# pgvector/pgvector

Measured on AMD Instinct MI355X. Metric: QPS @ recall@10 (IVFFlat, 1M x 1536d), higher is better.
Workload: dtype f32

## Files before the change

include/pgv_hip.h:

```cpp
#ifndef PGV_HIP_H
#define PGV_HIP_H

#include <stddef.h>
#include <stdint.h>

#ifdef __cplusplus
extern "C" {
#endif

#define PGV_ABI_VERSION 1

#define PGV_OK 0
#define PGV_ERR_ARG 1
#define PGV_ERR_DIMS 2
#define PGV_ERR_DEVICE 3
#define PGV_ERR_NOMEM 4
#define PGV_ERR_STATE 5
#define PGV_ERR_DATA 6

typedef enum pgv_dtype
{
	PGV_F32 = 0,
	PGV_F16 = 1
}			pgv_dtype;
// ... 51 lines not shown
	double		scan_pairs;
	double		scan_rows;
	double		aux_ms;
	int64_t		aux_launches;
	double		aux_pairs;
	double		assign_redo_rows;
	double		assign_rows;
	double		assign_recheck_rows;
	double		scan_unique_rows;
	double		scan_redo_queries;
	double		scan_widened_queries;
	double		scan_shadow_queries;
}			pgv_stats;
int			pgv_ctx_set_profiling(pgv_ctx * ctx, int on);
int			pgv_ctx_set_exact_scan(pgv_ctx * ctx, int on);
#define PGV_BOUND_STATISTICAL 0
#define PGV_BOUND_WORST_CASE 1
int			pgv_ctx_set_bound(pgv_ctx * ctx, int mode);
int			pgv_ctx_reset_stats(pgv_ctx * ctx);
int			pgv_ctx_get_stats(pgv_ctx * ctx, pgv_stats * out);


int			pgv_index_upload(pgv_ctx * ctx, pgv_metric metric, pgv_dtype dtype, int dim, int nlists,
							 const void *centers, const int64_t *list_offsets,
							 const void *vectors, const uint64_t *tids, pgv_index * *out);
void		pgv_index_free(pgv_index * index);
int			pgv_index_share(pgv_index * index, pgv_ctx * ctx, pgv_index * *out);
int			pgv_index_set_overlap(pgv_index * index, int lanes);
#define PGV_INDEX_HANDLE_BYTES 256
typedef struct pgv_index_handle
// ... 5 lines not shown
int			pgv_index_tids(pgv_index * index, const int64_t *slots, int64_t n, uint64_t *out);
int64_t		pgv_index_rows(const pgv_index * index);
int			pgv_index_lists(const pgv_index * index);

int			pgv_rank_lists(pgv_index * index, const void *queries, int nq, int maxprobes,
						   int32_t *out_lists, float *out_dist);

int			pgv_scan_lists(pgv_index * index, const void *query, const int32_t *lists, int nlists,
						   float *out_dist, int64_t *out_slot, int64_t capacity, int64_t *out_count);

int			pgv_search_batch(pgv_index * index, const void *queries, int nq, int probes, int k,
							 float *out_dist, int64_t *out_slot, uint64_t *out_tid);

int			pgv_index_shadow_cast(pgv_index * index, const void *queries, int nq, void *out_qcast, float *out_qscale,
								  float *out_qeps, float *out_cscale, float *out_ceps);

int			pgv_scan_batch(pgv_index * index, const void *queries, int nq, const int32_t *probe_lists,
						   int probes, int k, float *out_dist, int64_t *out_slot, uint64_t *out_tid);

typedef struct pgv_query pgv_query;
int			pgv_query_begin(pgv_index * index, pgv_query * *out);
void		pgv_query_end(pgv_query * q);
int			pgv_query_rank(pgv_query * q, const void *query, int max_probes);
int			pgv_query_scan(pgv_query * q, int first, int nprobes, int head, float *out_dist, int64_t *out_slot,
						   uint64_t *out_tid, int *out_count, int64_t *out_total);
int			pgv_query_more(pgv_query * q, int skip, int count, float *out_dist, int64_t *out_slot,
						   uint64_t *out_tid, int *out_count);
int			pgv_query_lists(pgv_query * q, int32_t *out_lists, int n);


// ... 158 lines not shown
```

pgvector_amd/_lib.py:

```python
import ctypes as C
import os

try:
    import torch
except ImportError:
    torch = None

_HERE = os.path.dirname(os.path.abspath(__file__))
LIB_PATH = os.environ.get("PGV_HIP_LIB") or os.path.join(_HERE, "lib", "libpgv_hip.so")

PGV_OK, PGV_ERR_ARG, PGV_ERR_DIMS, PGV_ERR_DEVICE, PGV_ERR_NOMEM, PGV_ERR_STATE, PGV_ERR_DATA = range(7)
PGV_F32, PGV_F16 = 0, 1
PGV_L2SQ, PGV_NEG_IP, PGV_L1 = 0, 1, 2
PGV_OPS_L2, PGV_OPS_IP, PGV_OPS_COSINE = 0, 1, 2
PGV_BOUND_STATISTICAL, PGV_BOUND_WORST_CASE = 0, 1

SYMBOLS = [
    "pgv_last_error", "pgv_abi_version", "pgv_device_count", "pgv_scan_chain_length", "pgv_ctx_create", "pgv_ctx_destroy",
    "pgv_ctx_sync", "pgv_ctx_stream", "pgv_timer_start", "pgv_timer_stop", "pgv_ctx_set_profiling", "pgv_ctx_set_exact_scan", "pgv_index_share", "pgv_pinned_alloc", "pgv_pinned_free",
    "pgv_ctx_reset_stats", "pgv_ctx_get_stats", "pgv_index_upload", "pgv_index_free",
    "pgv_index_rows", "pgv_index_lists", "pgv_rank_lists", "pgv_scan_lists", "pgv_search_batch", "pgv_scan_batch",
    "pgv_assign", "pgv_kmeans", "pgv_lloyd_partial", "pgv_lloyd_finish", "pgv_kmeanspp_init",
    "pgv_distance_batch", "pgv_cosine_distance_batch", "pgv_bit_distance_batch", "pgv_hnsw_upload", "pgv_hnsw_free", "pgv_hnsw_score", "pgv_hnsw_set_graph", "pgv_hnsw_search",
    "pgv_hnsw_build_search", "pgv_hnsw_build_neighbors", "pgv_hnsw_link_begin", "pgv_hnsw_link_prepare",
    "pgv_hnsw_link_apply", "pgv_hnsw_link_end", "pgv_hnsw_build_search_keep", "pgv_hnsw_build_select_kept", "pgv_hnsw_score_pairs", "pgv_hnsw_score_groups", "pgv_hnsw_update_graph",
    "pgv_query_begin", "pgv_query_end", "pgv_query_rank", "pgv_query_scan", "pgv_query_more", "pgv_query_lists",
    "pgv_comm_unique_id", "pgv_comm_create", "pgv_comm_create_custom", "pgv_comm_destroy", "pgv_comm_size",
    "pgv_comm_rank", "pgv_kmeans_sharded", "pgv_search_batch_sharded",
    "pgv_device_memory", "pgv_pinned_register", "pgv_pinned_unregister", "pgv_index_export", "pgv_index_import",
    "pgv_index_tids", "pgv_hnsw_export", "pgv_hnsw_import", "pgv_hnsw_share", "pgv_hnsw_device", "pgv_exact_topk", "pgv_ctx_set_bound",
    "pgv_hnsw_upload_payload", "pgv_hnsw_get_payload", "pgv_builder_begin", "pgv_builder_add", "pgv_builder_set_centers", "pgv_builder_rows", "pgv_builder_finish", "pgv_builder_free", "pgv_index_drain",
    "pgv_index_set_overlap", "pgv_index_shadow_cast", "pgv_bit_topk", "pgv_binary_quantize", "pgv_rerank",
    "pgv_hnsw_upload_bits", "pgv_index_upload_bits", "pgv_index_nbits", "pgv_bit_assign", "pgv_bit_kmeans",
    "pgv_bit_lloyd_step",
]


class PgvError(RuntimeError):
    def __init__(self, code, message):
        super().__init__("libpgv_hip error %d: %s" % (code, message))
        self.code = code
        self.message = message


class PgvStats(C.Structure):
    _fields_ = [("scan_ms", C.c_double), ("scan_launches", C.c_int64),
                ("scan_pairs", C.c_double), ("scan_rows", C.c_double),
# ... 30 lines not shown
    lib.pgv_last_error.argtypes = []
    lib.pgv_abi_version.restype = I
    lib.pgv_device_count.restype = I
    lib.pgv_scan_chain_length.argtypes = [I, I, I]
    lib.pgv_scan_chain_length.restype = I
    lib.pgv_ctx_create.argtypes = [I, P, C.POINTER(P)]
    lib.pgv_ctx_destroy.argtypes = [P]
    lib.pgv_ctx_destroy.restype = None
    lib.pgv_ctx_sync.argtypes = [P]
    lib.pgv_ctx_stream.argtypes = [P]
    lib.pgv_ctx_stream.restype = P
    lib.pgv_timer_start.argtypes = [P]
    lib.pgv_timer_stop.argtypes = [P, C.POINTER(C.c_float)]
    lib.pgv_ctx_set_profiling.argtypes = [P, I]
    lib.pgv_ctx_set_exact_scan.argtypes = [P, I]
    lib.pgv_ctx_reset_stats.argtypes = [P]
    lib.pgv_ctx_get_stats.argtypes = [P, C.POINTER(PgvStats)]
    lib.pgv_index_upload.argtypes = [P, I, I, I, I, P, P, P, P, C.POINTER(P)]
    lib.pgv_index_free.argtypes = [P]
    lib.pgv_index_share.argtypes = [P, P, C.POINTER(P)]
    lib.pgv_index_set_overlap.argtypes = [P, I]
    lib.pgv_index_shadow_cast.argtypes = [P, P, I, P, P, P, P, P]
    lib.pgv_index_free.restype = None
    lib.pgv_index_export.argtypes = [P, P]
    lib.pgv_index_import.argtypes = [P, P, C.POINTER(P)]
    lib.pgv_index_tids.argtypes = [P, P, I64, P]
    lib.pgv_hnsw_export.argtypes = [P, P]
    lib.pgv_hnsw_share.argtypes = [P, P, C.POINTER(P)]
    lib.pgv_hnsw_device.argtypes = [P]
    lib.pgv_hnsw_upload_payload.argtypes = [P, I, I, I, P, I64, P, I, C.POINTER(P)]
    lib.pgv_hnsw_get_payload.argtypes = [P, P, I, P]
    lib.pgv_hnsw_upload_bits.argtypes = [P, I, I, P, I64, P, I, C.POINTER(P)]
    lib.pgv_exact_topk.argtypes = [P, I, I, I, P, I, P, I64, I, P, P]
    lib.pgv_ctx_set_bound.argtypes = [P, I]
    lib.pgv_builder_begin.argtypes = [P, I, I, I, I, P, I64, C.POINTER(P)]
    lib.pgv_builder_add.argtypes = [P, P, P, I64]
    lib.pgv_builder_set_centers.argtypes = [P, P]
# ... 70 lines not shown
```

pgvector_amd/api.py:

```python
import ctypes as C
import weakref

import numpy as np

from . import _lib
from ._lib import (PGV_ERR_ARG, PGV_ERR_STATE, PGV_F16, PGV_F32, PGV_L1, PGV_L2SQ, PGV_NEG_IP, PGV_OPS_COSINE,
                   PGV_OPS_IP, PGV_OPS_L2, PgvError, PgvRng, PgvStats, check, lib)

_NP_OF = {PGV_F32: np.float32, PGV_F16: np.float16}


def _is_torch(x):
    return type(x).__module__.startswith("torch")


def ptr(x):
    if x is None:
        return None
    if _is_torch(x):
        assert x.is_contiguous(), "tensor must be contiguous"
        return C.c_void_p(x.data_ptr())
    assert isinstance(x, np.ndarray) and x.flags["C_CONTIGUOUS"], "need a C-contiguous array"
    return C.c_void_p(x.ctypes.data)

# ... 64 lines not shown
        return lib.pgv_ctx_stream(self.h)

    def timer_start(self):
        check(lib.pgv_timer_start(self.h))

    def timer_stop(self):
        ms = C.c_float()
        check(lib.pgv_timer_stop(self.h, C.byref(ms)))
        return ms.value

    def set_profiling(self, on):
        check(lib.pgv_ctx_set_profiling(self.h, 1 if on else 0))

    def set_exact_scan(self, on):
        check(lib.pgv_ctx_set_exact_scan(self.h, 1 if on else 0))

    def set_bound(self, worst_case):
        check(lib.pgv_ctx_set_bound(self.h, _lib.PGV_BOUND_WORST_CASE if worst_case else _lib.PGV_BOUND_STATISTICAL))

    def reset_stats(self):
        check(lib.pgv_ctx_reset_stats(self.h))

    def stats(self):
        s = PgvStats()
        check(lib.pgv_ctx_get_stats(self.h, C.byref(s)))
        return {"scan_ms": s.scan_ms, "scan_launches": s.scan_launches,
                "scan_pairs": s.scan_pairs, "scan_rows": s.scan_rows,
                "aux_ms": s.aux_ms, "aux_launches": s.aux_launches, "aux_pairs": s.aux_pairs,
                "assign_redo_rows": s.assign_redo_rows, "assign_rows": s.assign_rows,
                "assign_recheck_rows": s.assign_recheck_rows, "scan_unique_rows": s.scan_unique_rows, "scan_redo_queries": s.scan_redo_queries,
# ... 776 lines not shown
```

pgvector_amd/csrc/kernels_query.hip:

```cpp
#include "pgv_device.h"
#include "pgv_select.h"

#include <type_traits>

namespace pgv {

namespace {

constexpr int kQThreads = kSelThreads;
constexpr int kQWaves = kQThreads / kWave;
constexpr int kMaxBatchLists = 256;
constexpr int kHeadCap = 1024;

template <typename T, int METRIC, int NCH> struct WholeRows {
    Raw16 q[NCH];
    __device__ __forceinline__ void load_query(const char *qp, int lane) {
#pragma unroll
        for (int c = 0; c < NCH; c++) q[c] = load16(qp + ((size_t)c * kWave + lane) * sizeof(Raw16));
    }
    __device__ __forceinline__ float pair(const char *a, const char *b, int lane) const {
        Raw16 ra[NCH], rb[NCH];
#pragma unroll
        for (int c = 0; c < NCH; c++) ra[c] = load16(a + ((size_t)c * kWave + lane) * sizeof(Raw16));
#pragma unroll
// ... 92 lines not shown
        w.load_query(qp, lane);
        for (int64_t j = first + 2 * wave; j < end; j += 2 * kQWaves) {
            const bool two = j + 1 < end;
            const float d = w.pair(row_ptr(j), row_ptr(two ? j + 1 : j), lane);
            if (lane == 0 || (lane == 1 && two)) out[j + lane] = d;
        }
    } else {
        const int rpw = kWave >> lg;
        const int g = lane >> lg, lane_in = lane & ((1 << lg) - 1);
        for (int64_t j0 = first + (int64_t)wave * rpw; j0 < end; j0 += (int64_t)kQWaves * rpw) {
            const int64_t j = j0 + g;
            const bool valid = j < end;
            const float d = group_distance<T, METRIC>(row_ptr(valid ? j : end - 1), qp, nvec, lane_in, lg);
            if (valid && lane_in == (1 << lg) - 1) out[j] = d;
        }
    }
}

template <typename T, int METRIC, int NCH>
__global__ __launch_bounds__(kQThreads) void query_rank_kernel(const char *__restrict__ centers, int nlists, int nvec,
                                                               int lg, const char *__restrict__ qp,
                                                               float *__restrict__ cdist, int per) {
    const size_t row_bytes = (size_t)nvec * sizeof(Raw16);
    for (int64_t first = (int64_t)blockIdx.x * per; first < nlists; first += (int64_t)gridDim.x * per) {
        const int64_t end = first + per < nlists ? first + per : nlists;
        score_rows<T, METRIC, NCH>([&](int64_t j) { return centers + (size_t)j * row_bytes; }, first, end, qp, nvec, lg,
                                   cdist);
    }
}

// ... 168 lines not shown
        } else {
            out_dist[o] = INFINITY;
            if (out_slot) out_slot[o] = -1;
            if (out_tid) out_tid[o] = ~0ull;
        }
    }
    if (stats && threadIdx.x == 0) {
        atomicAdd(&stats[0], (double)m);
        atomicAdd(&stats[1], (double)m);
        atomicAdd(&stats[5], (double)m);
    }
}

constexpr int kRecheckCap = 256;

template <typename T, bool DOT = false>
__global__ __launch_bounds__(kQThreads) void batch_recheck_kernel(
    const char *__restrict__ vectors, const uint64_t *__restrict__ tids, int nvec, int lg,
    const char *__restrict__ queries, int kprime, int k, const float *__restrict__ approx_val,
    const int64_t *__restrict__ cand_pos, const int64_t *__restrict__ cand_slot,
    const int64_t *__restrict__ list_off, const int32_t *__restrict__ probe_lists,
    const int64_t *__restrict__ probe_off, int probes,
    const int64_t *__restrict__ seg_start, int64_t fixed_len,
    const unsigned *__restrict__ row_norm_max, ScanBound bound, const float *__restrict__ eps_add, int nq,
    float *__restrict__ out_dist, int64_t *__restrict__ out_slot, uint64_t *__restrict__ out_tid,
    int32_t *__restrict__ out_i32, int32_t *__restrict__ flags, float *__restrict__ pair_t, PlanEmit emit) {
    static_assert(!DOT || std::is_same<T, float>::value, "pair terms: fp32 rows");
    __shared__ float exact[kRecheckCap];
    __shared__ float dots[DOT ? kRecheckCap : 1];
    __shared__ __attribute__((aligned(16))) unsigned long long ent[kRecheckCap];
    const int q = blockIdx.x;
    const size_t row_bytes = (size_t)nvec * sizeof(Raw16);
    const int64_t m = seg_start ? seg_start[q + 1] - seg_start[q] : fixed_len;
    const int ncand = (int)(m < kprime ? m : (int64_t)kprime);
    const int kk = ncand < k ? ncand : k;
    const float *av = approx_val + (size_t)q * kprime;
    __shared__ float qn_part[kQWaves];
    {
        const char *qrow = queries + (size_t)q * row_bytes;
        float a = 0.f;
        for (int v = threadIdx.x; v < nvec; v += kQThreads) {
            const Raw16 x = load16(qrow + (size_t)v * sizeof(Raw16));
            a = accum_slice<T, 1>(a, x, x);
        }
        for (int m2 = 32; m2 > 0; m2 >>= 1) a += __shfl_xor(a, m2);
        if ((threadIdx.x & (kWave - 1)) == 0) qn_part[threadIdx.x >> 6] = a;
    }
    __syncthreads();
    float qn = 0.f;
    for (int w = 0; w < kQWaves; w++) qn += qn_part[w];
    const float rn = __uint_as_float(*row_norm_max);
    const float cross = 2.f * sqrtf(qn * rn);
    const float eps = 1.001f * (bound.g_sq * (qn + rn + cross) + bound.g_dot * cross + bound.g_norm * rn +
                                (eps_add ? eps_add[q] : 0.f));
    unsigned band = 0u;
    if (kk > 0) {
        const float edge = av[kk - 1] + 2.f * eps;
        band = float_to_key(edge + bound.g_ref * fabsf(edge + qn));
    }
    const int cnt = __syncthreads_count((int)threadIdx.x < ncand && float_to_key(av[threadIdx.x]) <= band);
    __shared__ int64_t slots[kRecheckCap];
    if ((int)threadIdx.x < cnt) {
        const int64_t p = cand_pos[(size_t)q * kprime + threadIdx.x];
        int64_t slot = p;
        if (cand_slot) {
            slot = cand_slot[(size_t)q * kprime + threadIdx.x];
        } else {
            const int64_t *off = probe_off + (size_t)q * probes;
            int lo = 0, hi = probes - 1;
            while (lo < hi) {
                const int mid = (lo + hi + 1) >> 1;
                if (off[mid] <= p)
                    lo = mid;
                else
                    hi = mid - 1;
            }
            slot = list_off[probe_lists[(size_t)q * probes + lo]] + (p - off[lo]);
        }
        slots[threadIdx.x] = slot;
    }
    __syncthreads();
    if constexpr (DOT)
        score_rows_dot([&](int64_t j) { return vectors + (size_t)slots[j] * row_bytes; }, 0, cnt,
                       queries + (size_t)q * row_bytes, nvec, lg, exact, dots);
    else
        score_rows<T, 0, 0>([&](int64_t j) { return vectors + (size_t)slots[j] * row_bytes; }, 0, cnt,
                            queries + (size_t)q * row_bytes, nvec, lg, exact);
    __syncthreads();
    if ((int)threadIdx.x < kRecheckCap)
        ent[threadIdx.x] = (int)threadIdx.x < cnt
                               ? ((unsigned long long)float_to_key(exact[threadIdx.x]) << 32) |
                                     (unsigned)cand_pos[(size_t)q * kprime + threadIdx.x]
                               : ~0ull;
    __syncthreads();
    const unsigned long long mine = ent[threadIdx.x];
    const int64_t my_slot = (int)threadIdx.x < cnt ? slots[threadIdx.x] : -1;
    int rank = 0;
    {
        const ulonglong2 *e2 = reinterpret_cast<const ulonglong2 *>(ent);
        const int n2 = (cnt + 1) / 2;
#pragma unroll 8
        for (int j = 0; j < n2; j++) {
            const ulonglong2 o = e2[j];
            rank += o.x < mine ? 1 : 0;
            rank += o.y < mine ? 1 : 0;
        }
    }
    if ((int)threadIdx.x < cnt && rank < k) {
        const size_t o = (size_t)q * k + rank;
        out_dist[o] = key_to_float((unsigned)(mine >> 32));
        if (out_slot) out_slot[o] = my_slot;
        if (out_i32) out_i32[o] = (int32_t)my_slot;
        if (out_tid) out_tid[o] = tids ? tids[my_slot] : ~0ull;
        if constexpr (DOT) pair_t[o] = -2.f * dots[threadIdx.x];
    }
    if ((int)threadIdx.x >= kk && (int)threadIdx.x < k) {
        const size_t o = (size_t)q * k + threadIdx.x;
        out_dist[o] = INFINITY;
        if (out_slot) out_slot[o] = -1;
        if (out_i32) out_i32[o] = -1;
        if (out_tid) out_tid[o] = ~0ull;
        if constexpr (DOT) pair_t[o] = 0.f;
    }
    if constexpr (DOT) {
        if (emit.cnt) {
            __syncthreads();
            if ((int)threadIdx.x < cnt && rank < k) {
                atomicAdd(&emit.cnt[my_slot], 1);
                slots[rank] = emit.list_off[my_slot + 1] - emit.list_off[my_slot];
            }
            if ((int)threadIdx.x >= kk && (int)threadIdx.x < k) slots[threadIdx.x] = 0;
            __syncthreads();
            if ((int)threadIdx.x < k) {
                int64_t run = 0;
                for (int i = 0; i < (int)threadIdx.x; i++) run += slots[i];
                emit.probe_off[(size_t)q * k + threadIdx.x] = run;
                if ((int)threadIdx.x == k - 1) emit.seg_len[q] = run + slots[threadIdx.x];
            }
        }
    }
    if (threadIdx.x == 0) {
        const int32_t flag = (m > ncand && cnt == ncand) ? 1 : 0;
        flags[q] = flag;
        if (flag) flags[nq + 1 + atomicAdd(&flags[nq], 1)] = q;
// ... 359 lines not shown
              : (t.fixed_len != 0 || !t.probe_off || !t.seg_start || t.probes < 1))
        PGV_FAIL(PGV_ERR_ARG, "exact tail: a list plan or one dense run");
    if (t.kprime > kRecheckCap || t.k > t.kprime)
        PGV_FAIL(PGV_ERR_ARG, "exact tail: k' = %d outside k..%d", t.kprime, kRecheckCap);
    if (t.pair_t && xr.dtype != PGV_F32) PGV_FAIL(PGV_ERR_ARG, "exact tail: pair terms are for fp32 rows");
    static_assert(kWide >= kRecheckCap, "k <= k' <= kWide: batch_fix_kernel's emit");
    if (t.emit.cnt && !(dense && t.pair_t && t.out_i32 && t.emit.probe_off && t.emit.seg_len && t.emit.list_off))
        PGV_FAIL(PGV_ERR_ARG, "exact tail: the plan is counted where the pair terms are written");
    ApproxScratch sc;
    PGV_TRY(sc.carve(scratch, t.nq, t.kprime));
    const int64_t *cand_slot = dense ? sc.cand_pos : nullptr;
    const int64_t *seg_start = dense ? nullptr : t.seg_start;
    const int64_t fixed_len = dense ? t.fixed_len : 0;
    PGV_TRY(launch_topk_segments(ctx, t.approx, seg_start, t.nq, fixed_len, t.kprime, sc.cand_val, sc.cand_pos,
                                 sc.flags + t.nq, t.emit.cnt, t.emit.cnt ? 2 * (int)fixed_len : 0));
#define PGV_RECHECK(T, DOT)                                                                                          \
    hipLaunchKernelGGL((batch_recheck_kernel<T, DOT>), dim3(t.nq), dim3(kQThreads), 0, ctx->stream,                   \
                       static_cast<const char *>(xr.vectors), xr.tids, xr.geom.nvec, xr.geom.lpr_log2,                \
                       static_cast<const char *>(t.queries), t.kprime, t.k, sc.cand_val, sc.cand_pos, cand_slot,      \
                       xr.list_offsets, t.probe_lists, t.probe_off, t.probes, seg_start, fixed_len, xr.norm_max,      \
                       t.bound, t.eps_add, t.nq, t.out_dist, t.out_slot, t.out_tid, t.out_i32, sc.flags, t.pair_t,    \
                       t.emit)
    if (t.pair_t)
        PGV_RECHECK(float, true);
    else if (xr.dtype == PGV_F32)
        PGV_RECHECK(float, false);
    else
        PGV_RECHECK(__half, false);
#undef PGV_RECHECK
    PGV_HIP(hipGetLastError());
    double *stats = (ctx->profiling && ctx->stats_dev.p) ? ctx->stats_dev.as<double>() : nullptr;
    int kp = 2;
    while (kp < t.k) kp <<= 1;
    const int cap = kp > kFastCap ? kp : kFastCap;
    const size_t lds = (size_t)cap * 8 + sizeof(SelShared);
    const int grid = t.nq < ctx->num_cus ? t.nq : ctx->num_cus;
#define PGV_FIX(T)                                                                                                    \
    hipLaunchKernelGGL(batch_fix_kernel<T>, dim3(grid), dim3(kQThreads), lds, ctx->stream,                            \
                       static_cast<const char *>(xr.vectors), xr.list_offsets, xr.tids, xr.geom.nvec,                 \
                       xr.geom.lpr_log2, static_cast<const char *>(t.queries), t.probe_lists, t.probe_off, t.probes,  \
                       seg_start, fixed_len, sc.flags, t.nq, t.approx, t.k, kp, cap, xr.norm_max, t.bound, t.eps_add, \
                       ctx->no_widen ? 0 : 1, t.out_dist, t.out_slot, t.out_tid, t.out_i32, stats, t.pair_t, t.emit)
    if (xr.dtype == PGV_F32)
        PGV_FIX(float);
// ... 9 lines not shown
```

pgvector_amd/csrc/pgv_abi.hip:

```cpp
#include "pgv_abi_common.h"




namespace pgv {

static thread_local char g_err[512] = "";

void set_error(const char *fmt, ...) {
    va_list ap;
    va_start(ap, fmt);
    vsnprintf(g_err, sizeof(g_err), fmt, ap);
    va_end(ap);
}

int DBuf::ensure(size_t bytes) {
    bytes += 64;
    if (bytes <= cap && p) return PGV_OK;
    if (p) {
        (void)hipFree(p);
        p = nullptr;
        cap = 0;
    }
    size_t want = bytes < 256 ? 256 : bytes;
// ... 202 lines not shown
    if (!ctx) PGV_FAIL(PGV_ERR_ARG, "ctx is NULL");
    PGV_TRY(resolve_events(ctx));
    ctx->profiling = on != 0;
    if (ctx->profiling && !ctx->stats_dev.p) {
        PGV_TRY(ctx->stats_dev.ensure(8 * sizeof(double)));
        PGV_HIP(hipMemsetAsync(ctx->stats_dev.p, 0, 8 * sizeof(double), ctx->stream));
    }
    for (pgv_ctx *c : ctx->children) PGV_TRY(pgv_ctx_set_profiling(c, on));
    return PGV_OK;
}

int pgv_ctx_set_exact_scan(pgv_ctx *ctx, int on) {
    if (!ctx) PGV_FAIL(PGV_ERR_ARG, "pgv_ctx_set_exact_scan: ctx is NULL");
    ctx->no_mfma_scan = on != 0;
    for (pgv_ctx *c : ctx->children) c->no_mfma_scan = ctx->no_mfma_scan;
    return PGV_OK;
}

int pgv_ctx_set_bound(pgv_ctx *ctx, int mode) {
    if (!ctx) PGV_FAIL(PGV_ERR_ARG, "pgv_ctx_set_bound: ctx is NULL");
    if (mode != PGV_BOUND_STATISTICAL && mode != PGV_BOUND_WORST_CASE)
        PGV_FAIL(PGV_ERR_ARG, "pgv_ctx_set_bound: unknown mode %d", mode);
    ctx->bound_mode = mode;
    ctx->assign_bound_mode = mode;
    for (pgv_ctx *c : ctx->children) c->bound_mode = c->assign_bound_mode = mode;
    return PGV_OK;
}

int pgv_ctx_reset_stats(pgv_ctx *ctx) {
    if (!ctx) PGV_FAIL(PGV_ERR_ARG, "ctx is NULL");
// ... 59 lines not shown
```

pgvector_amd/csrc/pgv_abi_ivf.hip:

```cpp
#include "pgv_abi_common.h"

extern "C" {


namespace {
struct IndexLayout {
    size_t centers, vectors, offsets, tids, row_norms, center_norms, bytes;
    bool has_tids, has_norms;
};
IndexLayout index_layout(int nlists, int64_t n, size_t row_bytes, bool has_tids, bool l2) {
    auto up = [](size_t v) { return (v + 255) & ~(size_t)255; };
    IndexLayout L{};
    size_t at = 0;
    L.centers = at; at = up(at + (size_t)nlists * row_bytes);
    L.vectors = at; at = up(at + (size_t)(n > 0 ? n : 1) * row_bytes);
    L.offsets = at; at = up(at + sizeof(int64_t) * ((size_t)nlists + 1));
    L.has_tids = has_tids;
    L.tids = at; if (has_tids) at = up(at + sizeof(uint64_t) * (size_t)n);
    L.has_norms = l2;
    L.row_norms = at; if (l2 && n > 0) at = up(at + sizeof(float) * ((size_t)n + 1));
    L.center_norms = at; if (l2) at = up(at + sizeof(float) * ((size_t)nlists + 1));
    L.bytes = at;
    return L;
}
// ... 96 lines not shown

struct ShadowBatch {
    void *qcast = nullptr;
    float *qscale = nullptr, *qeps = nullptr;
    float *cscale = nullptr, *ceps = nullptr;
    float *pair_t = nullptr;
    bool scan_follows = false;
    bool cast_for_scan = false;
    bool pairs_done = false;
};

int shadow_batch_cast(pgv_index *ix, const void *q_dev, int nq, int probes, bool for_rank, bool for_scan, ShadowBatch *sb) {
    pgv_ctx *ctx = ix->ctx;
    const RowGeom &g16 = ix->shadow_geom;
    const size_t qb = ((size_t)nq * g16.ld * sizeof(uint16_t) + 255) & ~(size_t)255;
    PGV_TRY(ctx->sh_q.ensure(qb + sizeof(float) * (size_t)nq * (4 + (size_t)probes)));
    sb->qcast = ctx->sh_q.p;
    sb->qscale = reinterpret_cast<float *>(ctx->sh_q.as<char>() + qb);
    sb->qeps = sb->qscale + nq;
    sb->cscale = sb->qeps + nq;
    sb->ceps = sb->cscale + nq;
    sb->pair_t = sb->ceps + nq;
    constexpr double u = 5.9604644775390625e-8;
    ShadowTerms st{};
    st.s = ix->shadow_s;
    st.E = ix->shadow_E;
    st.P = ix->shadow_P;
    st.g_dot = gamma_n(shadow_chain_length(g16) + 4.0, u);
    st.g_pair = gamma_n((double)pair_chain_length(ix->geom), u);
    st.g_cn = shadow_band(ix->geom.ld, 0.f, u).g_norm;
// ... 474 lines not shown
    index_drop_lanes(ix);
    if (lanes == 1) return PGV_OK;
    PGV_HIP(hipEventCreateWithFlags(&ix->lane_event, hipEventDisableTiming));
    PGV_HIP(hipEventCreateWithFlags(&ix->lane_scan_done, hipEventDisableTiming));
    for (int i = 0; i < lanes; i++) {
        pgv_ctx *lc = nullptr;
        pgv_index *v = nullptr;
        int rc = pgv_ctx_create(ix->ctx->device, nullptr, &lc);
        if (rc == PGV_OK) rc = pgv_index_share(ix, lc, &v);
        if (rc != PGV_OK) {
            if (lc) pgv_ctx_destroy(lc);
            index_drop_lanes(ix);
            return rc;
        }
        lc->no_mfma_scan = ix->ctx->no_mfma_scan;
        lc->bound_mode = ix->ctx->bound_mode;
        lc->assign_bound_mode = ix->ctx->assign_bound_mode;
        if (ix->ctx->profiling) (void)pgv_ctx_set_profiling(lc, 1);
        lc->scan_gate = ix->lane_scan_done;
        ix->lanes.push_back(v);
        ix->ctx->children.push_back(lc);
    }
    return PGV_OK;
}

int pgv_index_share(pgv_index *ix, pgv_ctx *ctx, pgv_index **out) {
    if (!ix || !ctx || !out) PGV_FAIL(PGV_ERR_ARG, "pgv_index_share: index/ctx/out is NULL");
    *out = nullptr;
    if (ctx->device != ix->ctx->device)
        PGV_FAIL(PGV_ERR_ARG, "pgv_index_share: the index lives on device %d, the context on %d", ix->ctx->device, ctx->device);
// ... 226 lines not shown
        tail.rows = {ix->centers, nullptr, nullptr, ix->geom, ix->dtype,
                     reinterpret_cast<const unsigned *>(ix->center_norms + ix->nlists)};
        tail.queries = q_dev;
        tail.nq = nq;
        tail.kprime = cand;
        tail.k = maxprobes;
        tail.approx = mat;
        tail.fixed_len = ix->nlists;
        tail.bound = scan_bound_chain(ctx, ix->geom.ld, scan_chain_length(ix->geom, ix->dtype, false));
        if (rank_sh) tail.bound = shadow_band(ix->geom.ld, tail.bound.g_ref);
        tail.eps_add = rank_sh ? sb->ceps : nullptr;
        tail.out_dist = dist;
        tail.out_i32 = out_lists_dev;
        PGV_TRY(launch_exact_tail(ctx, tail, ctx->ms_b));
        sb->pairs_done = tail.pair_t != nullptr;
        return PGV_OK;
    } else {
        PGV_TRY(dense_scan(ctx, ix->metric, ix->dtype, ix->geom, ix->centers, ix->nlists, q_dev, nq, ix->nlists, mat,
                           mfma, nullptr, nullptr));
        PGV_TRY(launch_topk_segments(ctx, mat, nullptr, nq, ix->nlists, maxprobes, dist, pos));
    }
    PGV_TRY(launch_cast_pos_to_i32(ctx, pos, (int64_t)nq * maxprobes, out_lists_dev));
    return PGV_OK;
}

int rank_lists_dev(pgv_index *ix, const void *q_dev, int nq, int maxprobes, int32_t *out_lists_dev, float *out_dist_dev) {
    return rank_lists_impl(ix, q_dev, nq, maxprobes, out_lists_dev, out_dist_dev, nullptr);
}

int pgv_rank_lists(pgv_index *ix, const void *queries, int nq, int maxprobes, int32_t *out_lists,
// ... 339 lines not shown
    const struct {
        void *dst;
        const void *src;
        size_t bytes;
    } parts[] = {{out_qcast, sb.qcast, (size_t)nq * ix->shadow_geom.ld * sizeof(uint16_t)},
                 {out_qscale, sb.qscale, sizeof(float) * (size_t)nq},
                 {out_qeps, sb.qeps, sizeof(float) * (size_t)nq},
                 {out_cscale, sb.cscale, sizeof(float) * (size_t)nq},
                 {out_ceps, sb.ceps, sizeof(float) * (size_t)nq}};
    for (const auto &p : parts)
        if (p.dst) PGV_HIP(hipMemcpyAsync(p.dst, p.src, p.bytes, hipMemcpyDefault, ctx->stream));
    PGV_HIP(hipStreamSynchronize(ctx->stream));
    return PGV_OK;
}

namespace {

struct QueryHeadHost {
    long long total;
    int count;
    unsigned seq;
};

static int g_scan_gate_width = -1;
static PgvGate g_scan_gate;
static void scan_gate_enter() {
    if (g_scan_gate_width < 0) {
        const char *e = getenv("PGV_MAX_INFLIGHT_SCANS");
        __atomic_store_n(&g_scan_gate_width, e ? atoi(e) : 16, __ATOMIC_RELAXED);
    }
// ... 189 lines not shown
```

pgvector_amd/csrc/pgv_internal.h:

```cpp
#pragma once

#include <hip/hip_runtime.h>

#include <cstdint>
#include <cstdio>
#include <cstdlib>
#include <cstring>
#include <cmath>
#include <vector>

#include "../../include/pgv_hip.h"

namespace pgv {

void set_error(const char *fmt, ...) __attribute__((format(printf, 1, 2)));

#define PGV_FAIL(code, ...)            \
    do {                               \
        ::pgv::set_error(__VA_ARGS__); \
        return (code);                 \
    } while (0)

#define PGV_HIP(call)                                                                  \
    do {                                                                               \
// ... 92 lines not shown
    int device = 0;
    hipStream_t stream = nullptr;
    bool own_stream = false;
    int num_cus = 256;
    hipEvent_t ev0 = nullptr, ev1 = nullptr;
    pgv::DBuf q_stage, rows_stage, centers_stage, out_stage, out_stage2, idx_stage;
    pgv::DBuf tasks, pairs, counters, plan_a, plan_b, plan_c, plan_d, dist_mat, sel_a, sel_b;
    pgv::DBuf km_a, km_b, km_c, km_d, km_e, km_f, km_g;
    pgv::DBuf ms_b;
    pgv::DBuf dense_plan;
    int64_t dense_plan_rows = -1, dense_plan_stride = -1;
    int dense_plan_nq = -1, dense_plan_kind = -1;
    bool counters_clean = false;
    pgv::DBuf ms_a;
    pgv::DBuf sh_q;
    pgv::DBuf mf_d;
    pgv::DBuf mf_a, mf_b, mf_c, zeros;
    pgv::DBuf stats_dev;
    pgv::HBuf h_a, h_b, h_c;
    hipEvent_t h_a_busy = nullptr;
    bool h_a_pending = false;
    bool profiling = false;
    bool no_mfma_scan = false;
    bool no_widen = false;
    int bound_mode = 1;
    int assign_bound_mode = 1;
    pgv::DBuf xt_norms;
    std::vector<hipEvent_t> ev_pool;
    size_t ev_used = 0;
    double scan_ms = 0.0;
    int64_t scan_launches = 0;
    double scan_pairs = 0.0;
    double scan_rows = 0.0;
    std::vector<char> ev_is_aux;
    double aux_ms = 0.0;
    int64_t aux_launches = 0;
    double aux_pairs = 0.0;
    double scan_shadow_queries = 0.0;
// ... 415 lines not shown
```

Baseline: 1.372 million.

## Add software-pipelined gather path to batch recheck kernel with staged probe offsets

Adds a GATHER variant of the batch recheck kernel, on by default. It loads candidate rows in register-batched steps separated by scheduling barriers so memory loads overlap scoring. It preloads per-thread candidate values, positions and norms, stages probe offsets and lists in shared memory for the binary search, and overlaps the tid and list-length fetches with the first row loads. It also sets a waves-per-EU occupancy hint and adds an API to toggle the path and to read back the last pair terms. The larger register and shared-memory footprint could lower occupancy.

Result: faster. 1.386 million, median of 6 (+1.0%).

```diff
diff --git a/include/pgv_hip.h b/include/pgv_hip.h
--- a/include/pgv_hip.h
+++ b/include/pgv_hip.h
@@ -89,6 +89,7 @@
 }			pgv_stats;
 int			pgv_ctx_set_profiling(pgv_ctx * ctx, int on);
 int			pgv_ctx_set_exact_scan(pgv_ctx * ctx, int on);
+int			pgv_ctx_set_recheck_gather(pgv_ctx * ctx, int on);
 #define PGV_BOUND_STATISTICAL 0
 #define PGV_BOUND_WORST_CASE 1
 int			pgv_ctx_set_bound(pgv_ctx * ctx, int mode);
@@ -124,6 +125,7 @@
 
 int			pgv_index_shadow_cast(pgv_index * index, const void *queries, int nq, void *out_qcast, float *out_qscale,
 								  float *out_qeps, float *out_cscale, float *out_ceps);
+int			pgv_ctx_last_pair_terms(pgv_ctx * ctx, float *out, int64_t n);
 
 int			pgv_scan_batch(pgv_index * index, const void *queries, int nq, const int32_t *probe_lists,
 						   int probes, int k, float *out_dist, int64_t *out_slot, uint64_t *out_tid);
diff --git a/pgvector_amd/_lib.py b/pgvector_amd/_lib.py
--- a/pgvector_amd/_lib.py
+++ b/pgvector_amd/_lib.py
@@ -17,7 +17,7 @@
 
 SYMBOLS = [
     "pgv_last_error", "pgv_abi_version", "pgv_device_count", "pgv_scan_chain_length", "pgv_ctx_create", "pgv_ctx_destroy",
-    "pgv_ctx_sync", "pgv_ctx_stream", "pgv_timer_start", "pgv_timer_stop", "pgv_ctx_set_profiling", "pgv_ctx_set_exact_scan", "pgv_index_share", "pgv_pinned_alloc", "pgv_pinned_free",
+    "pgv_ctx_sync", "pgv_ctx_stream", "pgv_timer_start", "pgv_timer_stop", "pgv_ctx_set_profiling", "pgv_ctx_set_exact_scan", "pgv_ctx_set_recheck_gather", "pgv_index_share", "pgv_pinned_alloc", "pgv_pinned_free",
     "pgv_ctx_reset_stats", "pgv_ctx_get_stats", "pgv_index_upload", "pgv_index_free",
     "pgv_index_rows", "pgv_index_lists", "pgv_rank_lists", "pgv_scan_lists", "pgv_search_batch", "pgv_scan_batch",
     "pgv_assign", "pgv_kmeans", "pgv_lloyd_partial", "pgv_lloyd_finish", "pgv_kmeanspp_init",
@@ -30,7 +30,7 @@
     "pgv_device_memory", "pgv_pinned_register", "pgv_pinned_unregister", "pgv_index_export", "pgv_index_import",
     "pgv_index_tids", "pgv_hnsw_export", "pgv_hnsw_import", "pgv_hnsw_share", "pgv_hnsw_device", "pgv_exact_topk", "pgv_ctx_set_bound",
     "pgv_hnsw_upload_payload", "pgv_hnsw_get_payload", "pgv_builder_begin", "pgv_builder_add", "pgv_builder_set_centers", "pgv_builder_rows", "pgv_builder_finish", "pgv_builder_free", "pgv_index_drain",
-    "pgv_index_set_overlap", "pgv_index_shadow_cast", "pgv_bit_topk", "pgv_binary_quantize", "pgv_rerank",
+    "pgv_index_set_overlap", "pgv_index_shadow_cast", "pgv_ctx_last_pair_terms", "pgv_bit_topk", "pgv_binary_quantize", "pgv_rerank",
     "pgv_hnsw_upload_bits", "pgv_index_upload_bits", "pgv_index_nbits", "pgv_bit_assign", "pgv_bit_kmeans",
     "pgv_bit_lloyd_step",
 ]
@@ -91,6 +91,7 @@
     lib.pgv_timer_stop.argtypes = [P, C.POINTER(C.c_float)]
     lib.pgv_ctx_set_profiling.argtypes = [P, I]
     lib.pgv_ctx_set_exact_scan.argtypes = [P, I]
+    lib.pgv_ctx_set_recheck_gather.argtypes = [P, I]
     lib.pgv_ctx_reset_stats.argtypes = [P]
     lib.pgv_ctx_get_stats.argtypes = [P, C.POINTER(PgvStats)]
     lib.pgv_index_upload.argtypes = [P, I, I, I, I, P, P, P, P, C.POINTER(P)]
@@ -98,6 +99,7 @@
     lib.pgv_index_share.argtypes = [P, P, C.POINTER(P)]
     lib.pgv_index_set_overlap.argtypes = [P, I]
     lib.pgv_index_shadow_cast.argtypes = [P, P, I, P, P, P, P, P]
+    lib.pgv_ctx_last_pair_terms.argtypes = [P, P, C.c_int64]
     lib.pgv_index_free.restype = None
     lib.pgv_index_export.argtypes = [P, P]
     lib.pgv_index_import.argtypes = [P, P, C.POINTER(P)]
diff --git a/pgvector_amd/api.py b/pgvector_amd/api.py
--- a/pgvector_amd/api.py
+++ b/pgvector_amd/api.py
@@ -102,6 +102,9 @@
 
     def set_exact_scan(self, on):
         check(lib.pgv_ctx_set_exact_scan(self.h, 1 if on else 0))
+
+    def set_recheck_gather(self, on):
+        check(lib.pgv_ctx_set_recheck_gather(self.h, 1 if on else 0))
 
     def set_bound(self, worst_case):
         check(lib.pgv_ctx_set_bound(self.h, _lib.PGV_BOUND_WORST_CASE if worst_case else _lib.PGV_BOUND_STATISTICAL))
diff --git a/pgvector_amd/csrc/kernels_query.hip b/pgvector_amd/csrc/kernels_query.hip
--- a/pgvector_amd/csrc/kernels_query.hip
+++ b/pgvector_amd/csrc/kernels_query.hip
@@ -130,6 +130,94 @@
             const float d = group_distance<T, METRIC>(row_ptr(valid ? j : end - 1), qp, nvec, lane_in, lg);
             if (valid && lane_in == (1 << lg) - 1) out[j] = d;
         }
+    }
+}
+
+template <typename T, bool DOT, int NCH, int R, typename RowPtr, typename Extra>
+__device__ __forceinline__ void gather_rows(RowPtr row_ptr, int cnt, const char *qp, int nvec, int lg, float *out,
+                                            float *out_dot, Extra extra) {
+    const int lane = threadIdx.x & (kWave - 1);
+    const int wave = threadIdx.x >> 6;
+    const int lpr = 1 << lg, rpw = kWave >> lg;
+    const int g = lane >> lg, lane_in = lane & (lpr - 1);
+    const int stride = kQWaves * rpw;
+    if (wave * rpw >= cnt) {
+        extra();
+        return;
+    }
+    unsigned voff[NCH];
+#pragma unroll
+    for (int c = 0; c < NCH; c++) {
+        const int v = lane_in + c * lpr;
+        voff[c] = (unsigned)(v < nvec ? v : 0) * (unsigned)sizeof(Raw16);
+    }
+    Raw16 qv[NCH], x[R][NCH];
+    auto load_step = [&](int j0) {
+#pragma unroll
+        for (int r = 0; r < R; r++) {
+            const int j = j0 + r * stride + g;
+            const char *row = row_ptr(j < cnt ? j : cnt - 1);
+#pragma unroll
+            for (int c = 0; c < NCH; c++) x[r][c] = load16(row + voff[c]);
+        }
+    };
+    auto score_step = [&](int j0) {
+#pragma unroll
+        for (int r = 0; r < R; r++) {
+            float acc[2] = {0.f, 0.f}, dot[2] = {0.f, 0.f};
+#pragma unroll
+            for (int c = 0; c < NCH; c++) {
+                const bool in_row = lane_in + c * lpr < nvec;
+                const float a = accum_slice<T, 0>(acc[c & 1], x[r][c], qv[c]);
+                acc[c & 1] = in_row ? a : acc[c & 1];
+                asm("" : "+v"(acc[c & 1]));
+                if constexpr (DOT) {
+                    const float b = accum_slice<T, 1>(dot[c & 1], x[r][c], qv[c]);
+                    dot[c & 1] = in_row ? b : dot[c & 1];
+                    asm("" : "+v"(dot[c & 1]));
+                }
+            }
+            const float d = finish<0>(group_sum_to_last(acc[0] + acc[1], lg));
+            float qx = 0.f;
+            if constexpr (DOT) qx = group_sum_to_last(dot[0] + dot[1], lg);
+            const int j = j0 + r * stride + g;
+            if (j < cnt && lane_in == lpr - 1) {
+                out[j] = d;
+                if constexpr (DOT) out_dot[j] = qx;
+            }
+        }
+    };
+    int j0 = wave * rpw;
+#pragma unroll
+    for (int c = 0; c < NCH; c++) qv[c] = load16(qp + voff[c]);
+    load_step(j0);
+    extra();
+    __builtin_amdgcn_sched_barrier(0);
+    score_step(j0);
+    for (j0 += R * stride; j0 < cnt; j0 += R * stride) {
+        load_step(j0);
+        __builtin_amdgcn_sched_barrier(0);
+        score_step(j0);
+    }
+}
+
+constexpr int kGatherMaxTrips = 8;
+template <typename T, bool DOT, typename RowPtr, typename Extra>
+__device__ __forceinline__ void gather_rows_any(RowPtr row_ptr, int cnt, const char *qp, int nvec, int lg, float *out,
+                                                float *out_dot, Extra extra) {
+    const int nch = (nvec + (1 << lg) - 1) >> lg;
+    if (nch <= 2) {
+        gather_rows<T, DOT, 2, 4>(row_ptr, cnt, qp, nvec, lg, out, out_dot, extra);
+    } else if (nch <= 6) {
+        gather_rows<T, DOT, 6, 2>(row_ptr, cnt, qp, nvec, lg, out, out_dot, extra);
+    } else if (!DOT && nch <= kGatherMaxTrips) {
+        gather_rows<T, false, kGatherMaxTrips, 1>(row_ptr, cnt, qp, nvec, lg, out, out_dot, extra);
+    } else {
+        extra();
+        if constexpr (DOT)
+            score_rows_dot(row_ptr, 0, cnt, qp, nvec, lg, out, out_dot);
+        else
+            score_rows<T, 0, 0>(row_ptr, 0, cnt, qp, nvec, lg, out);
     }
 }
 
@@ -328,8 +416,10 @@
 
 constexpr int kRecheckCap = 256;
 
-template <typename T, bool DOT = false>
-__global__ __launch_bounds__(kQThreads) void batch_recheck_kernel(
+constexpr int kStageProbes = 1024;
+
+template <typename T, bool DOT = false, bool GATHER = true>
+__global__ __launch_bounds__(kQThreads) __attribute__((amdgpu_waves_per_eu(4, 8))) void batch_recheck_kernel(
     const char *__restrict__ vectors, const uint64_t *__restrict__ tids, int nvec, int lg,
     const char *__restrict__ queries, int kprime, int k, const float *__restrict__ approx_val,
     const int64_t *__restrict__ cand_pos, const int64_t *__restrict__ cand_slot,
@@ -350,7 +440,60 @@
     const int kk = ncand < k ? ncand : k;
     const float *av = approx_val + (size_t)q * kprime;
     __shared__ float qn_part[kQWaves];
-    {
+    __shared__ float edge_av;
+    __shared__ int64_t st_off[GATHER ? kStageProbes : 1];
+    __shared__ int32_t st_pl[GATHER ? kStageProbes : 1];
+    const bool staged = GATHER && !cand_slot && probes <= kStageProbes;
+    float my_av = 0.f, my_rn = 0.f, my_eps_add = 0.f;
+    int64_t my_pos = 0, my_given = 0;
+    if constexpr (GATHER) {
+        const char *qrow = queries + (size_t)q * row_bytes;
+        my_rn = __uint_as_float(*row_norm_max);
+        my_eps_add = eps_add ? eps_add[q] : 0.f;
+        const size_t mine = (size_t)q * kprime + ((int)threadIdx.x < kprime ? threadIdx.x : kprime - 1);
+        my_av = approx_val[mine];
+        my_pos = cand_pos[mine];
+        my_given = (cand_slot ? cand_slot : cand_pos)[mine];
+        constexpr int kPer = kStageProbes / kQThreads;
+        int64_t so[kPer] = {};
+        int32_t sp[kPer] = {};
+        if (staged) {
+#pragma unroll
+            for (int i = 0; i < kPer; i++) {
+                const int e = threadIdx.x + i * kQThreads;
+                so[i] = probe_off[(size_t)q * probes + (e < probes ? e : 0)];
+                sp[i] = probe_lists[(size_t)q * probes + (e < probes ? e : 0)];
+            }
+        }
+        float a = 0.f;
+        for (int v0 = threadIdx.x; v0 < nvec; v0 += 4 * kQThreads) {
+            Raw16 x[4];
+#pragma unroll
+            for (int i = 0; i < 4; i++) {
+                const int v = v0 + i * kQThreads;
+                x[i] = load16(qrow + (size_t)(v < nvec ? v : v0) * sizeof(Raw16));
+            }
+            __builtin_amdgcn_sched_barrier(0);
+#pragma unroll
+            for (int i = 0; i < 4; i++) {
+                const float b = accum_slice<T, 1>(a, x[i], x[i]);
+                a = v0 + i * kQThreads < nvec ? b : a;
+            }
+        }
+        for (int m2 = 32; m2 > 0; m2 >>= 1) a += __shfl_xor(a, m2);
+        if ((threadIdx.x & (kWave - 1)) == 0) qn_part[threadIdx.x >> 6] = a;
+        if ((int)threadIdx.x == kk - 1) edge_av = my_av;
+        if (staged) {
+#pragma unroll
+            for (int i = 0; i < kPer; i++) {
+                const int e = threadIdx.x + i * kQThreads;
+                if (e < probes) {
+                    st_off[e] = so[i];
+                    st_pl[e] = sp[i];
+                }
+            }
+        }
+    } else {
         const char *qrow = queries + (size_t)q * row_bytes;
         float a = 0.f;
         for (int v = threadIdx.x; v < nvec; v += kQThreads) {
@@ -363,38 +506,63 @@
     __syncthreads();
     float qn = 0.f;
     for (int w = 0; w < kQWaves; w++) qn += qn_part[w];
-    const float rn = __uint_as_float(*row_norm_max);
+    const float rn = GATHER ? my_rn : __uint_as_float(*row_norm_max);
     const float cross = 2.f * sqrtf(qn * rn);
     const float eps = 1.001f * (bound.g_sq * (qn + rn + cross) + bound.g_dot * cross + bound.g_norm * rn +
-                                (eps_add ? eps_add[q] : 0.f));
+                                (GATHER ? my_eps_add : (eps_add ? eps_add[q] : 0.f)));
     unsigned band = 0u;
     if (kk > 0) {
-        const float edge = av[kk - 1] + 2.f * eps;
+        const float edge = (GATHER ? edge_av : av[kk - 1]) + 2.f * eps;
         band = float_to_key(edge + bound.g_ref * fabsf(edge + qn));
     }
-    const int cnt = __syncthreads_count((int)threadIdx.x < ncand && float_to_key(av[threadIdx.x]) <= band);
+    const int cnt = __syncthreads_count((int)threadIdx.x < ncand &&
+                                        float_to_key(GATHER ? my_av : av[threadIdx.x]) <= band);
     __shared__ int64_t slots[kRecheckCap];
+    int64_t my_slot = -1;
     if ((int)threadIdx.x < cnt) {
-        const int64_t p = cand_pos[(size_t)q * kprime + threadIdx.x];
+        const int64_t p = GATHER ? my_pos : cand_pos[(size_t)q * kprime + threadIdx.x];
         int64_t slot = p;
         if (cand_slot) {
-            slot = cand_slot[(size_t)q * kprime + threadIdx.x];
+            slot = GATHER ? my_given : cand_slot[(size_t)q * kprime + threadIdx.x];
         } else {
             const int64_t *off = probe_off + (size_t)q * probes;
             int lo = 0, hi = probes - 1;
-            while (lo < hi) {
-                const int mid = (lo + hi + 1) >> 1;
-                if (off[mid] <= p)
-                    lo = mid;
-                else
-                    hi = mid - 1;
-            }
-            slot = list_off[probe_lists[(size_t)q * probes + lo]] + (p - off[lo]);
+            if (staged) {
+                while (lo < hi) {
+                    const int mid = (lo + hi + 1) >> 1;
+                    if (st_off[mid] <= p)
+                        lo = mid;
+                    else
+                        hi = mid - 1;
+                }
+                slot = list_off[st_pl[lo]] + (p - st_off[lo]);
+            } else {
+                while (lo < hi) {
+                    const int mid = (lo + hi + 1) >> 1;
+                    if (off[mid] <= p)
+                        lo = mid;
+                    else
+                        hi = mid - 1;
+                }
+                slot = list_off[probe_lists[(size_t)q * probes + lo]] + (p - off[lo]);
+            }
         }
         slots[threadIdx.x] = slot;
+        my_slot = slot;
     }
     __syncthreads();
-    if constexpr (DOT)
+    uint64_t my_tid = ~0ull;
+    int64_t my_len = 0;
+    if constexpr (GATHER)
+        gather_rows_any<T, DOT>([&](int64_t j) { return vectors + (size_t)slots[j] * row_bytes; }, cnt,
+                                queries + (size_t)q * row_bytes, nvec, lg, exact, dots, [&]() {
+                                    if ((int)threadIdx.x < cnt) {
+                                        if (out_tid && tids) my_tid = tids[my_slot];
+                                        if constexpr (DOT)
+                                            if (emit.cnt) my_len = emit.list_off[my_slot + 1] - emit.list_off[my_slot];
+                                    }
+                                });
+    else if constexpr (DOT)
         score_rows_dot([&](int64_t j) { return vectors + (size_t)slots[j] * row_bytes; }, 0, cnt,
                        queries + (size_t)q * row_bytes, nvec, lg, exact, dots);
     else
@@ -404,11 +572,10 @@
     if ((int)threadIdx.x < kRecheckCap)
         ent[threadIdx.x] = (int)threadIdx.x < cnt
                                ? ((unsigned long long)float_to_key(exact[threadIdx.x]) << 32) |
-                                     (unsigned)cand_pos[(size_t)q * kprime + threadIdx.x]
+                                     (unsigned)(GATHER ? my_pos : cand_pos[(size_t)q * kprime + threadIdx.x])
                                : ~0ull;
     __syncthreads();
     const unsigned long long mine = ent[threadIdx.x];
-    const int64_t my_slot = (int)threadIdx.x < cnt ? slots[threadIdx.x] : -1;
     int rank = 0;
     {
         const ulonglong2 *e2 = reinterpret_cast<const ulonglong2 *>(ent);
@@ -425,7 +592,7 @@
         out_dist[o] = key_to_float((unsigned)(mine >> 32));
         if (out_slot) out_slot[o] = my_slot;
         if (out_i32) out_i32[o] = (int32_t)my_slot;
-        if (out_tid) out_tid[o] = tids ? tids[my_slot] : ~0ull;
+        if (out_tid) out_tid[o] = GATHER ? my_tid : (tids ? tids[my_slot] : ~0ull);
         if constexpr (DOT) pair_t[o] = -2.f * dots[threadIdx.x];
     }
     if ((int)threadIdx.x >= kk && (int)threadIdx.x < k) {
@@ -441,7 +608,7 @@
             __syncthreads();
             if ((int)threadIdx.x < cnt && rank < k) {
                 atomicAdd(&emit.cnt[my_slot], 1);
-                slots[rank] = emit.list_off[my_slot + 1] - emit.list_off[my_slot];
+                slots[rank] = GATHER ? my_len : emit.list_off[my_slot + 1] - emit.list_off[my_slot];
             }
             if ((int)threadIdx.x >= kk && (int)threadIdx.x < k) slots[threadIdx.x] = 0;
             __syncthreads();
@@ -831,8 +998,15 @@
     const int64_t fixed_len = dense ? t.fixed_len : 0;
     PGV_TRY(launch_topk_segments(ctx, t.approx, seg_start, t.nq, fixed_len, t.kprime, sc.cand_val, sc.cand_pos,
                                  sc.flags + t.nq, t.emit.cnt, t.emit.cnt ? 2 * (int)fixed_len : 0));
-#define PGV_RECHECK(T, DOT)                                                                                          \
-    hipLaunchKernelGGL((batch_recheck_kernel<T, DOT>), dim3(t.nq), dim3(kQThreads), 0, ctx->stream,                   \
+#define PGV_RECHECK(T, DOT)               \
+    do {                                  \
+        if (ctx->no_recheck_gather)       \
+            PGV_RECHECK_(T, DOT, false);  \
+        else                              \
+            PGV_RECHECK_(T, DOT, true);   \
+    } while (0)
+#define PGV_RECHECK_(T, DOT, GATHER)                                                                                 \
+    hipLaunchKernelGGL((batch_recheck_kernel<T, DOT, GATHER>), dim3(t.nq), dim3(kQThreads), 0, ctx->stream,           \
                        static_cast<const char *>(xr.vectors), xr.tids, xr.geom.nvec, xr.geom.lpr_log2,                \
                        static_cast<const char *>(t.queries), t.kprime, t.k, sc.cand_val, sc.cand_pos, cand_slot,      \
                        xr.list_offsets, t.probe_lists, t.probe_off, t.probes, seg_start, fixed_len, xr.norm_max,      \
@@ -845,6 +1019,7 @@
     else
         PGV_RECHECK(__half, false);
 #undef PGV_RECHECK
+#undef PGV_RECHECK_
     PGV_HIP(hipGetLastError());
     double *stats = (ctx->profiling && ctx->stats_dev.p) ? ctx->stats_dev.as<double>() : nullptr;
     int kp = 2;
diff --git a/pgvector_amd/csrc/pgv_abi.hip b/pgvector_amd/csrc/pgv_abi.hip
--- a/pgvector_amd/csrc/pgv_abi.hip
+++ b/pgvector_amd/csrc/pgv_abi.hip
@@ -240,6 +240,13 @@
     if (!ctx) PGV_FAIL(PGV_ERR_ARG, "pgv_ctx_set_exact_scan: ctx is NULL");
     ctx->no_mfma_scan = on != 0;
     for (pgv_ctx *c : ctx->children) c->no_mfma_scan = ctx->no_mfma_scan;
+    return PGV_OK;
+}
+
+int pgv_ctx_set_recheck_gather(pgv_ctx *ctx, int on) {
+    if (!ctx) PGV_FAIL(PGV_ERR_ARG, "pgv_ctx_set_recheck_gather: ctx is NULL");
+    ctx->no_recheck_gather = on == 0;
+    for (pgv_ctx *c : ctx->children) c->no_recheck_gather = ctx->no_recheck_gather;
     return PGV_OK;
 }
 
diff --git a/pgvector_amd/csrc/pgv_abi_ivf.hip b/pgvector_amd/csrc/pgv_abi_ivf.hip
--- a/pgvector_amd/csrc/pgv_abi_ivf.hip
+++ b/pgvector_amd/csrc/pgv_abi_ivf.hip
@@ -134,6 +134,8 @@
     pgv_ctx *ctx = ix->ctx;
     const RowGeom &g16 = ix->shadow_geom;
     const size_t qb = ((size_t)nq * g16.ld * sizeof(uint16_t) + 255) & ~(size_t)255;
+    ctx->last_pair_t = nullptr;
+    ctx->last_pair_n = 0;
     PGV_TRY(ctx->sh_q.ensure(qb + sizeof(float) * (size_t)nq * (4 + (size_t)probes)));
     sb->qcast = ctx->sh_q.p;
     sb->qscale = reinterpret_cast<float *>(ctx->sh_q.as<char>() + qb);
@@ -638,6 +640,7 @@
             return rc;
         }
         lc->no_mfma_scan = ix->ctx->no_mfma_scan;
+        lc->no_recheck_gather = ix->ctx->no_recheck_gather;
         lc->bound_mode = ix->ctx->bound_mode;
         lc->assign_bound_mode = ix->ctx->assign_bound_mode;
         if (ix->ctx->profiling) (void)pgv_ctx_set_profiling(lc, 1);
@@ -894,6 +897,10 @@
         tail.out_i32 = out_lists_dev;
         PGV_TRY(launch_exact_tail(ctx, tail, ctx->ms_b));
         sb->pairs_done = tail.pair_t != nullptr;
+        if (sb->pairs_done) {
+            ctx->last_pair_t = tail.pair_t;
+            ctx->last_pair_n = (int64_t)nq * maxprobes;
+        }
         return PGV_OK;
     } else {
         PGV_TRY(dense_scan(ctx, ix->metric, ix->dtype, ix->geom, ix->centers, ix->nlists, q_dev, nq, ix->nlists, mat,
@@ -1263,6 +1270,17 @@
     return PGV_OK;
 }
 
+int pgv_ctx_last_pair_terms(pgv_ctx *ctx, float *out, int64_t n) {
+    if (!ctx || !out) PGV_FAIL(PGV_ERR_ARG, "pgv_ctx_last_pair_terms: ctx/out is NULL");
+    if (!ctx->last_pair_t || n != ctx->last_pair_n)
+        PGV_FAIL(PGV_ERR_STATE, "pgv_ctx_last_pair_terms: the last batch left %lld pair terms, %lld asked for",
+                 (long long)ctx->last_pair_n, (long long)n);
+    PGV_HIP(hipSetDevice(ctx->device));
+    PGV_HIP(hipMemcpyAsync(out, ctx->last_pair_t, sizeof(float) * (size_t)n, hipMemcpyDefault, ctx->stream));
+    PGV_HIP(hipStreamSynchronize(ctx->stream));
+    return PGV_OK;
+}
+
 namespace {
 
 struct QueryHeadHost {
diff --git a/pgvector_amd/csrc/pgv_internal.h b/pgvector_amd/csrc/pgv_internal.h
--- a/pgvector_amd/csrc/pgv_internal.h
+++ b/pgvector_amd/csrc/pgv_internal.h
@@ -130,6 +130,8 @@
     bool counters_clean = false;
     pgv::DBuf ms_a;
     pgv::DBuf sh_q;
+    const float *last_pair_t = nullptr;
+    int64_t last_pair_n = 0;
     pgv::DBuf mf_d;
     pgv::DBuf mf_a, mf_b, mf_c, zeros;
     pgv::DBuf stats_dev;
@@ -138,6 +140,7 @@
     bool h_a_pending = false;
     bool profiling = false;
     bool no_mfma_scan = false;
+    bool no_recheck_gather = false;
     bool no_widen = false;
     int bound_mode = 1;
     int assign_bound_mode = 1;
```
